# stattlab/azplugins

Hardware: AMD Instinct MI355X
Metric: particle-steps/sec, PerturbedLennardJones pair force (higher is better)
Workload: dtype f64

## Files before the change

### azplugins_amd/csrc/azp_device.hpp

```cpp
#pragma once

#include <hip/hip_runtime.h>
#include <stdint.h>

#include "../../include/azp.h"

namespace azp
{
constexpr int WAVE = 64;

struct BoxDev
    {
    double Lx, Ly, Lz;
    double Lxinv, Lyinv, Lzinv;
    double xy, xz, yz;
    int px, py, pz;
    int triclinic;
    };

inline BoxDev make_box_dev(const azp_box& b)
    {
    BoxDev d;
    d.Lx = b.L[0]; d.Ly = b.L[1]; d.Lz = b.L[2];
    d.Lxinv = 1.0 / b.L[0]; d.Lyinv = 1.0 / b.L[1]; d.Lzinv = 1.0 / b.L[2];
// ... 116 lines not shown
    {
    if (TPP >= 2) v += dpp_move<0xB1>(v);
    if (TPP >= 4) v += dpp_move<0x4E>(v);
    if (TPP >= 8) v += dpp_move<0x141>(v);
    if (TPP >= 16) v += dpp_move<0x140>(v);
    if (TPP >= 32) v += __shfl_xor(v, 16, WAVE);
    if (TPP >= 64) v += __shfl_xor(v, 32, WAVE);
    return v;
    }

__device__ __forceinline__ uint32_t wave_inclusive_scan(uint32_t v)
    {
    const uint32_t lane = threadIdx.x & (WAVE - 1);
#pragma unroll
    for (uint32_t d = 1; d < WAVE; d <<= 1)
        {
        const uint32_t up = (uint32_t)__shfl_up((int)v, d, WAVE);
        if (lane >= d)
            v += up;
        }
    return v;
    }

template<uint32_t NW> __device__ __forceinline__ uint32_t block_exclusive_scan(uint32_t mine, uint32_t* s_wave, uint32_t& total)
    {
    const uint32_t lane = threadIdx.x & (WAVE - 1), wave = threadIdx.x / WAVE;
    const uint32_t incl = wave_inclusive_scan(mine);
    if (lane == WAVE - 1)
        s_wave[wave] = incl;
    __syncthreads();
    uint32_t before = 0;
    total = 0;
#pragma unroll
    for (uint32_t w = 0; w < NW; ++w)
        {
        const uint32_t x = s_wave[w];
        before += (w < wave) ? x : 0u;
        total += x;
        }
    return before + (incl - mine);
    }

__device__ __forceinline__ double fast_rcp(double a)
    {
    const double x = __builtin_amdgcn_rcp(a);
    const double e = __builtin_fma(-a, x, 1.0);
    const double t = __builtin_fma(e, e, e);
    return __builtin_fma(x, t, x);
    }

__device__ __forceinline__ double fast_rcp1(double a)
    {
    const double x = __builtin_amdgcn_rcp(a);
    const double e = __builtin_fma(-a, x, 1.0);
    return __builtin_fma(x, e, x);
    }

__device__ __forceinline__ double fast_rsqrt(double a)
    {
    const double y = __builtin_amdgcn_rsq(a);
    const double h = __builtin_fma(-a * y, y, 1.0);
    return __builtin_fma(y * h, __builtin_fma(0.375, h, 0.5), y);
    }
__device__ __forceinline__ double fast_sqrt(double a)
    {
    const double s = a * fast_rsqrt(a);
    return (a > 0.0) ? s : 0.0;
    }

template<class T> __device__ __forceinline__ T to_uniform(const T& v)
    {
    static_assert(sizeof(T) % 4 == 0, "to_uniform needs whole dwords");
    constexpr int W = sizeof(T) / 4;
    uint32_t w[W];
    __builtin_memcpy(w, &v, sizeof(T));
#pragma unroll
    for (int i = 0; i < W; ++i)
        w[i] = (uint32_t)__builtin_amdgcn_readfirstlane((int)w[i]);
    T r;
    __builtin_memcpy(&r, w, sizeof(T));
    return r;
    }

__device__ __forceinline__ uint32_t xcd_remap(uint32_t b, uint32_t nblocks_padded8)
    {
    const uint32_t per_xcd = nblocks_padded8 >> 3;
    return (b & 7u) * per_xcd + (b >> 3);
    }

}
```

### azplugins_amd/csrc/pair_kernel.hpp

```cpp
#pragma once

#include <type_traits>

#include "evaluators.hpp"
#include "pair_kernel_host.hpp"

namespace azp
{
struct PairKArgs
    {
    double* force;
    double* virial;
    uint64_t virial_pitch;
    const double* pos;
    const uint32_t* n_neigh;
    const uint32_t* nlist;
    const uint64_t* head_list;
    const double* rcutsq;
    const double* ronsq;
    BoxDev box;
    double r_list_max;
    uint32_t N;
    uint32_t ntypes;
    uint32_t shift_mode;
    uint32_t nblocks_padded;
    uint32_t first;
    uint32_t end;
    };

template<class E> __device__ __forceinline__ typename E::Coeff
prepare_coeff(const PairKArgs& a, const typename E::Params* params, uint32_t tp)
    {
    const double rcutsq = a.rcutsq[tp];
    bool energy_shift = (a.shift_mode == AZP_SHIFT_SHIFT);
    if (a.shift_mode == AZP_SHIFT_XPLOR && a.ronsq[tp] > rcutsq)
        energy_shift = true;
    return E::prepare(params[tp], rcutsq, energy_shift);
    }

inline int validate_pair_args(const azp_pair_args* args, const void* d_params)
    {
    if (!args || !d_params) return AZP_ERROR_INVALID_ARGUMENT;
    if (args->N == 0) return 1;
    if (!args->d_force || !args->d_pos || !args->d_n_neigh || !args->d_nlist || !args->d_head_list || !args->d_rcutsq)
        return AZP_ERROR_INVALID_ARGUMENT;
    if (args->ntypes == 0 || args->shift_mode > AZP_SHIFT_XPLOR) return AZP_ERROR_INVALID_ARGUMENT;
    if (args->shift_mode == AZP_SHIFT_XPLOR && !args->d_ronsq) return AZP_ERROR_INVALID_ARGUMENT;
    if (args->compute_virial && (!args->d_virial || args->virial_pitch < args->N)) return AZP_ERROR_INVALID_ARGUMENT;
    if (args->n_max < args->N) return AZP_ERROR_INVALID_ARGUMENT;
    if (args->block_size && (args->block_size % 64 || args->block_size > 256)) return AZP_ERROR_INVALID_ARGUMENT;
    if (args->range_count && (uint64_t)args->range_first + args->range_count > args->N) return AZP_ERROR_INVALID_ARGUMENT;
    return 0;
    }

struct ForceEnergy
    {
    struct Acc
        {
        double fx, fy, fz, pe;
        };
    static __device__ __forceinline__ void zero(Acc& a) { a.fx = a.fy = a.fz = a.pe = 0.0; }
    template<int TPP> static __device__ __forceinline__ void reduce(Acc& a)
        {
        a.fx = group_sum<TPP>(a.fx);
        a.fy = group_sum<TPP>(a.fy);
        a.fz = group_sum<TPP>(a.fz);
        a.pe = group_sum<TPP>(a.pe);
        }
    template<class KExtra> static __device__ __forceinline__ void store(const Acc& a, const PairKArgs& p, const KExtra&, uint32_t idx)
        {
        store_scalar4(p.force, idx, a.fx, a.fy, a.fz, 0.5 * a.pe);
        }
    };

template<class E, bool XPLOR = false> struct XIso : ForceEnergy
    {
    typedef typename E::Params Params;
    struct Coeff
        {
        typename E::Coeff c;
        double ronsq;
        };
    struct KExtra {};
    struct Own {};
    static constexpr int kExtra = 0;
    static constexpr bool kTag = false;
    static __device__ __forceinline__ Coeff prepare(const Params* params, const PairKArgs& a, uint32_t t, const KExtra&)
        {
        Coeff c;
        c.c = prepare_coeff<E>(a, params, t);
        c.ronsq = XPLOR ? a.ronsq[t] : 0.0;
        return c;
        }
    static __device__ __forceinline__ void load_own(const KExtra&, uint32_t, Own&) {}
    static __device__ __forceinline__ void load_extra(const KExtra&, uint32_t, const double*, uint32_t&) {}
    static __device__ __forceinline__ bool in_range(const Coeff&, double) { return true; }
    template<bool VIRIAL>
    static __device__ __forceinline__ void pair(const Coeff& c, const KExtra&, const Own&, double dx, double dy, double dz, double rsq,
                                                const double*, uint32_t, Acc& a, double (&v)[6])
        {
        double force_divr, pair_eng;
        const bool evaluated = E::eval(c.c, rsq, force_divr, pair_eng);
        if (XPLOR && evaluated)
            apply_xplor(rsq, c.ronsq, c.c.rcutsq, force_divr, pair_eng);
        a.fx = __builtin_fma(dx, force_divr, a.fx);
        a.fy = __builtin_fma(dy, force_divr, a.fy);
        a.fz = __builtin_fma(dz, force_divr, a.fz);
        a.pe += pair_eng;
        if (VIRIAL)
            {
            const double fxx = force_divr * dx, fyy = force_divr * dy;
            v[0] = __builtin_fma(fxx, dx, v[0]);
            v[1] = __builtin_fma(fxx, dy, v[1]);
            v[2] = __builtin_fma(fxx, dz, v[2]);
            v[3] = __builtin_fma(fyy, dy, v[3]);
            v[4] = __builtin_fma(fyy, dz, v[4]);
            v[5] = __builtin_fma(force_divr * dz, dz, v[5]);
            }
// ... 219 lines not shown
```

### azplugins_amd/csrc/pair_plj.hip

```cpp
#include "pair_auto.hpp"

extern "C" int azp_pair_forces_perturbed_lennard_jones(const azp_pair_args* args, const azp_plj_params* d_params, void* stream)
    {
    return azp::launch_policy_entry<azp::XIso<azp::EvalPLJ>>(args, d_params, stream);
    }

extern "C" int azp_pair_forces_planned_perturbed_lennard_jones(azp_pair_plan* plan, const azp_pair_args* args,
                                                const azp_plj_params* d_params, void* stream)
    {
    return azp::launch_policy_planned<azp::XIso<azp::EvalPLJ>>(plan, args, d_params, stream);
    }

#ifdef AZP_TIMELINE
namespace azp { __device__ unsigned long long g_timeline[8 * 4 * 16384]; }
extern "C" int azp_debug_timeline(unsigned long long* out, size_t n_words)
    {
    return (int)hipMemcpyFromSymbol(out, HIP_SYMBOL(azp::g_timeline), n_words * sizeof(unsigned long long));
    }
#endif
```

### azplugins_amd/csrc/pair_tiled.hpp

```cpp
#pragma once

#include <type_traits>

#include "pair_kernel.hpp"
#include "pair_plan.hpp"

#ifndef AZP_TILED_WAVES_PER_SIMD
#define AZP_TILED_WAVES_PER_SIMD 4
#endif

namespace azp
{
#ifdef AZP_TIMELINE
extern __device__ unsigned long long g_timeline[8 * 4 * 16384];
#endif

struct TileDyn
    {
    uint32_t n_shells;
    uint32_t stale;
    };

struct TiledKArgs
    {
    PairKArgs p;
    const uint32_t* tile_nstage;
    const uint64_t* tile_head;
    const uint32_t* stage_idx;
    const uint32_t* slice_Kend;
    uint32_t n_shells;
    const uint64_t* slice_head;
    const uint4* cnl;
    const uint8_t* perm;
    const TileDyn* dyn;
    const uint32_t* dflag;
    const unsigned long long* dbits;
    const float* disp;
    double shell_w;
    double shell_winv;
    double bound_extra;
    };

__device__ __forceinline__ float wave_max_nonneg(float v)
    {
#pragma unroll
    for (int off = 32; off > 0; off >>= 1)
        v = fmaxf(v, __shfl_xor(v, off, 64));
    return v;
    }

__device__ __forceinline__ uint32_t tile_shells_for(double b, double shell_winv)
    {
    if (!(b >= 0.0))
        return PLAN_SHELLS;
    if (b == 0.0)
        return 0u;
    if (!(shell_winv > 0.0))
        return PLAN_SHELLS;
    const double n = ceil(2.0 * b * (1.0 + 1e-9) * shell_winv);
    return n >= (double)PLAN_SHELLS ? PLAN_SHELLS : (uint32_t)n;
    }

#define AZP_TILE_STRIDE(CAP) ((CAP) + 1)

constexpr int TILE_BATCH = 4;

struct TileBatch
    {
    double x[TILE_BATCH], y[TILE_BATCH], z[TILE_BATCH];
    uint32_t off[TILE_BATCH];
    };

inline void fill_local_bound(TiledKArgs& k, const PairPlan& plan, const azp_pair_args& args)
    {
    const bool local = args.d_displacement && args.has_displacement_bound && args.displacement_bound >= 0.0;
    k.disp = local ? args.d_displacement : nullptr;
    k.dflag = (args.d_stale_flag && args.d_displacement_sq_bits) ? args.d_stale_flag : nullptr;
    k.dbits = k.dflag ? args.d_displacement_sq_bits : nullptr;
    if (k.dflag)
        k.disp = nullptr;
    k.shell_w = plan.shell_width;
    k.shell_winv = plan.shell_width > 0.0 ? 1.0 / plan.shell_width : 0.0;
    k.bound_extra = args.displacement_bound_extra > 0.0 ? args.displacement_bound_extra : 0.0;
    }

template<int CAP, int H> __device__ __forceinline__ void tile_gather(TileBatch& b, const uint4& u, const char* bx)
    {
    constexpr int NB = TILE_BATCH;
    const uint32_t w0 = H ? u.z : u.x, w1 = H ? u.w : u.y;
    b.off[0] = w0 & 0xffffu;
    b.off[1] = w0 >> 16;
    b.off[2] = w1 & 0xffffu;
    b.off[3] = w1 >> 16;
#pragma unroll
    for (int e = 0; e < NB; ++e)
        {
        b.x[e] = *reinterpret_cast<const double*>(bx + b.off[e]);
// ... 10 lines not shown
                                             double& fz, double& pe, double (&v)[6], uint32_t& n_core, uint32_t& n_in, double (&es)[2])
    {
    typedef typename E::Coeff Coeff;
    constexpr int NB = TILE_BATCH;
    constexpr bool SPLIT = SINGLE && !XPLOR && E::kSplitEnergy;
    double dx[NB], dy[NB], dz[NB], rsq[NB];
    bool any_in = false;
#pragma unroll
    for (int e = 0; e < NB; ++e)
        {
        dx[e] = pi.x - b.x[e]; dy[e] = pi.y - b.y[e]; dz[e] = pi.z - b.z[e];
        if (WRAP)
            min_image(a.p.box, dx[e], dy[e], dz[e]);
        rsq[e] = __builtin_fma(dz[e], dz[e], __builtin_fma(dy[e], dy[e], dx[e] * dx[e]));
        if (WRAP)
            rsq[e] = (b.off[e] == 0) ? 1.0e60 : rsq[e];
        any_in = any_in || (rsq[e] < rcutsq_max);
        }
    const bool none_in = !__any(any_in);
    if (SPLIT ? __builtin_expect(none_in, 0) : none_in)
        return;
    double fd[NB];
    if constexpr (SPLIT)
        {
        double x[NB];
        E::rcp4(rsq, x);
        bool any_core = false;
#pragma unroll
        for (int e = 0; e < NB; ++e)
            any_core = any_core || E::in_core(c0, rsq[e]);
        if (!__any(any_core))
            {
            const bool count_in = c0.tail_add != 0.0;
#pragma unroll
            for (int e = 0; e < NB; ++e)
                E::eval_split_tail(c0, rsq[e], x[e], fd[e], es[0], es[1], n_in, count_in);
            }
        else
            {
#pragma unroll
            for (int e = 0; e < NB; ++e)
                E::eval_split(c0, rsq[e], x[e], fd[e], pe, n_core, n_in);
            }
        }
#pragma unroll
    for (int e = 0; e < NB; ++e)
        {
        double force_divr, pair_eng = 0.0;
        if constexpr (SPLIT)
            force_divr = fd[e];
        else if (SINGLE)
            {
            const bool evaluated = E::eval(c0, rsq[e], force_divr, pair_eng);
            if (XPLOR && evaluated)
                apply_xplor(rsq[e], ronsq0, c0.rcutsq, force_divr, pair_eng);
            }
        else
            {
            const int typej = *reinterpret_cast<const int*>(bt + (b.off[e] >> 1));
            const uint32_t tp = (uint32_t)typei * a.p.ntypes + (uint32_t)typej;
            const Coeff cc = s_coeff[tp];
            const bool evaluated = E::eval(cc, rsq[e], force_divr, pair_eng);
            if (XPLOR && evaluated)
                apply_xplor(rsq[e], s_ronsq[tp], cc.rcutsq, force_divr, pair_eng);
            }
        fx = __builtin_fma(dx[e], force_divr, fx);
        fy = __builtin_fma(dy[e], force_divr, fy);
        fz = __builtin_fma(dz[e], force_divr, fz);
        if constexpr (!SPLIT)
            pe += pair_eng;
        if (VIRIAL)
            {
            const double fxx = force_divr * dx[e], fyy = force_divr * dy[e];
            v[0] = __builtin_fma(fxx, dx[e], v[0]);
            v[1] = __builtin_fma(fxx, dy[e], v[1]);
            v[2] = __builtin_fma(fxx, dz[e], v[2]);
            v[3] = __builtin_fma(fyy, dy[e], v[3]);
            v[4] = __builtin_fma(fyy, dz[e], v[4]);
            v[5] = __builtin_fma(force_divr * dz[e], dz[e], v[5]);
            }
        }
    }

template<class E, int TPP, int CAP, bool VIRIAL, bool SINGLE, bool XPLOR, bool WRAP>
__device__ __forceinline__ void tiled_loop(const TiledKArgs& a, const char* bx, const char* bt,
                                           const typename E::Coeff* __restrict__ s_coeff,
                                           const double* __restrict__ s_ronsq, const typename E::Coeff& c0, double ronsq0,
                                           double rcutsq_max, const char* __restrict__ slice_base, uint32_t lane_off, uint32_t Kb,
                                           double3 pi, int typei, double& fx, double& fy, double& fz, double& pe, double (&v)[6], uint32_t& n_core,
                                           uint32_t& n_in, double (&es)[2])
    {
    const uint4 zero4 = make_uint4(0, 0, 0, 0);
    auto chunk_at = [&](uint32_t kk) -> uint4
        { return *reinterpret_cast<const uint4*>(slice_base + (uint64_t)kk * 1024u + lane_off); };
    const uint32_t K = Kb >> 1;
    const uint32_t Kc = (Kb + 1u) >> 1;
    uint4 u = (Kc > 0) ? chunk_at(0) : zero4;
    uint4 un = (Kc > 1) ? chunk_at(1) : u;
    TileBatch A, B;
    tile_gather<CAP, 0>(A, u, bx);
    for (uint32_t kk = 0; kk < K; ++kk)
        {
        const uint4 un2 = chunk_at((kk + 2 < Kc) ? kk + 2 : Kc - 1);
        tile_gather<CAP, 1>(B, u, bx);
        __builtin_amdgcn_sched_barrier(0);
        tile_compute<E, CAP, VIRIAL, SINGLE, XPLOR, WRAP>(A, a, bt, s_coeff, s_ronsq, c0, ronsq0, rcutsq_max, pi, typei, fx, fy, fz, pe, v, n_core, n_in, es);
        __builtin_amdgcn_sched_barrier(0);
        tile_gather<CAP, 0>(A, un, bx);
        __builtin_amdgcn_sched_barrier(0);
        tile_compute<E, CAP, VIRIAL, SINGLE, XPLOR, WRAP>(B, a, bt, s_coeff, s_ronsq, c0, ronsq0, rcutsq_max, pi, typei, fx, fy, fz, pe, v, n_core, n_in, es);
        __builtin_amdgcn_sched_barrier(0);
        u = un;
        un = un2;
        }
    if (Kb & 1u)
        tile_compute<E, CAP, VIRIAL, SINGLE, XPLOR, WRAP>(A, a, bt, s_coeff, s_ronsq, c0, ronsq0, rcutsq_max, pi, typei, fx, fy, fz, pe, v, n_core, n_in, es);
    }

template<class E, int TPP, int CAP, bool VIRIAL, bool SINGLE, bool XPLOR>
__global__ void __launch_bounds__(256, E::kTileWaves) pair_forces_tiled_kernel(const TiledKArgs a, const typename E::Params* __restrict__ params)
    {
    typedef typename E::Coeff Coeff;
    constexpr int TB = 256 / TPP;
    constexpr int PW = 64 / TPP;
    extern __shared__ __attribute__((aligned(16))) unsigned char s_raw[];
    double* s_x = reinterpret_cast<double*>(s_raw);
    double* s_y = s_x + AZP_TILE_STRIDE(CAP);
    double* s_z = s_y + AZP_TILE_STRIDE(CAP);
    int* s_t = reinterpret_cast<int*>(s_z + AZP_TILE_STRIDE(CAP));
    Coeff* s_coeff = reinterpret_cast<Coeff*>(s_raw + (size_t)AZP_TILE_STRIDE(CAP) * 24 + (SINGLE ? 0 : (size_t)CAP * 4 + 8));
    double* s_ronsq = reinterpret_cast<double*>(s_coeff + (SINGLE ? 0 : a.p.ntypes * a.p.ntypes));

    const uint32_t tid = threadIdx.x;
    __builtin_amdgcn_s_setprio(3);
#ifdef AZP_TIMELINE
    const unsigned long long tl_t0 = __builtin_amdgcn_s_memrealtime();
    const unsigned long long tl_c0 = __builtin_amdgcn_s_memtime();
    unsigned long long tl_tb = 0, tl_tc = 0, tl_td = 0, tl_ta = 0;
#endif
    const uint32_t tile = a.p.first / TB + xcd_remap(blockIdx.x, a.p.nblocks_padded);
    const uint32_t first = tile * TB;
    if (first >= a.p.end)
        return;
    if (a.dyn && a.dyn->stale)
        return;
    if (a.dflag && *a.dflag)
        return;

    Coeff c0;
    double ronsq0 = 0.0;
    double rcutsq_max = 0.0;
    if (SINGLE)
        {
        c0 = to_uniform(prepare_coeff<E>(a.p, params, 0));
        if (XPLOR)
            ronsq0 = a.p.ronsq[0];
        rcutsq_max = c0.rcutsq;
        }
    else
        {
        const uint32_t ntp = a.p.ntypes * a.p.ntypes;
        for (uint32_t t = tid; t < ntp; t += 256)
            {
            s_coeff[t] = prepare_coeff<E>(a.p, params, t);
            s_ronsq[t] = XPLOR ? a.p.ronsq[t] : 0.0;
            }
        for (uint32_t t = 0; t < ntp; ++t)
            rcutsq_max = fmax(rcutsq_max, a.p.rcutsq[t]);
        }

#ifdef AZP_TIMELINE
    tl_ta = __builtin_amdgcn_s_memrealtime();
#endif
    const uint32_t n_stage = a.tile_nstage[tile];
    const uint32_t* __restrict__ stage = a.stage_idx + a.tile_head[tile];
    const double3 c = load_scalar3_of4(a.p.pos, first);
    if (tid == 0)
        {
        s_x[0] = PLAN_FAR; s_y[0] = PLAN_FAR; s_z[0] = PLAN_FAR;
        if (!SINGLE) s_t[0] = 0;
        }
    const uint32_t wave = (uint32_t)__builtin_amdgcn_readfirstlane((int)(tid >> 6)), lane = tid & 63;
    const uint32_t pl = lane / TPP;
    const uint32_t idx = first + ((TPP == 1 && a.perm) ? (uint32_t)a.perm[(uint64_t)tile * 256u + tid] : wave * PW + pl);
    const bool active = idx < a.p.end;
    const double4 own = load_scalar4(a.p.pos, active ? idx : first);
    const bool no_hint = !(a.p.r_list_max > 0.0);
    bool far_from_c = false;
    float dmax = a.disp ? a.disp[active ? idx : first] : 0.f;
    {
    constexpr int ROUNDS = (CAP + 255) / 256;
    uint32_t sj[ROUNDS];
#pragma unroll
    for (int r = 0; r < ROUNDS; ++r)
        {
        const uint32_t sidx = (uint32_t)r * 256u + tid;
        sj[r] = (sidx < n_stage) ? stage[sidx] : first;
        }
#ifdef AZP_TIMELINE
    __builtin_amdgcn_s_waitcnt(0);
    tl_tb = __builtin_amdgcn_s_memrealtime();
#endif
    double sxv[ROUNDS], syv[ROUNDS], szv[ROUNDS];
    int stv[ROUNDS];
    if (a.disp)
        {
#pragma unroll
        for (int r = 0; r < ROUNDS; ++r)
            dmax = fmaxf(dmax, a.disp[sj[r]]);
        }
#pragma unroll
    for (int r = 0; r < ROUNDS; ++r)
        {
        if (SINGLE)
            {
            const double3 pj = load_scalar3_of4(a.p.pos, sj[r]);
            sxv[r] = pj.x; syv[r] = pj.y; szv[r] = pj.z;
            }
        else
            {
            const double4 pj = load_scalar4(a.p.pos, sj[r]);
            sxv[r] = pj.x; syv[r] = pj.y; szv[r] = pj.z;
            stv[r] = type_from_w(pj.w);
            }
        }
#ifdef AZP_TIMELINE
    __builtin_amdgcn_s_waitcnt(0);
    tl_tc = __builtin_amdgcn_s_memrealtime();
#endif
#pragma unroll
    for (int r = 0; r < ROUNDS; ++r)
        {
        const uint32_t sidx = (uint32_t)r * 256u + tid;
        if (sidx < n_stage)
            {
            double x = sxv[r], y = syv[r], z = szv[r];
            if (!a.p.box.triclinic)
                {
                if (a.p.box.px) x = __builtin_fma(-a.p.box.Lx, rint((x - c.x) * a.p.box.Lxinv), x);
                if (a.p.box.py) y = __builtin_fma(-a.p.box.Ly, rint((y - c.y) * a.p.box.Lyinv), y);
                if (a.p.box.pz) z = __builtin_fma(-a.p.box.Lz, rint((z - c.z) * a.p.box.Lzinv), z);
                if (no_hint)
                    far_from_c = far_from_c || (a.p.box.px && fabs(x - c.x) >= 0.25 * a.p.box.Lx)
                                 || (a.p.box.py && fabs(y - c.y) >= 0.25 * a.p.box.Ly)
                                 || (a.p.box.pz && fabs(z - c.z) >= 0.25 * a.p.box.Lz);
                }
            s_x[sidx + 1] = x; s_y[sidx + 1] = y; s_z[sidx + 1] = z;
            if (!SINGLE)
                s_t[sidx + 1] = stv[r];
            }
        }
    }

    double3 pi = make_double3(0.0, 0.0, 0.0);
    int typei = 0;
    bool lane_wide = far_from_c || a.p.box.triclinic;
    if (active)
        {
        const double4 p = own;
        double x = p.x, y = p.y, z = p.z;
        if (!a.p.box.triclinic)
            {
            if (a.p.box.px) x = __builtin_fma(-a.p.box.Lx, rint((x - c.x) * a.p.box.Lxinv), x);
            if (a.p.box.py) y = __builtin_fma(-a.p.box.Ly, rint((y - c.y) * a.p.box.Lyinv), y);
            if (a.p.box.pz) z = __builtin_fma(-a.p.box.Lz, rint((z - c.z) * a.p.box.Lzinv), z);
            const double rx = no_hint ? 0.25 * a.p.box.Lx : a.p.r_list_max, ry = no_hint ? 0.25 * a.p.box.Ly : a.p.r_list_max,
                         rz = no_hint ? 0.25 * a.p.box.Lz : a.p.r_list_max;
            lane_wide = lane_wide || (a.p.box.px && fabs(x - c.x) + rx >= 0.5 * a.p.box.Lx)
                        || (a.p.box.py && fabs(y - c.y) + ry >= 0.5 * a.p.box.Ly)
                        || (a.p.box.pz && fabs(z - c.z) + rz >= 0.5 * a.p.box.Lz);
            }
        pi = make_double3(x, y, z);
        typei = type_from_w(p.w);
        }
#ifdef AZP_TIMELINE
    __builtin_amdgcn_s_waitcnt(0);
    tl_td = __builtin_amdgcn_s_memrealtime();
#endif
    __shared__ float s_dmax[4];
    if (a.disp)
        {
        dmax = wave_max_nonneg(dmax);
        if (lane == 0)
            s_dmax[wave] = dmax;
        }
    const bool wide = __syncthreads_or(lane_wide);
    __builtin_amdgcn_s_setprio(0);
#ifdef AZP_TIMELINE
    const unsigned long long tl_t1 = __builtin_amdgcn_s_memrealtime();
#endif
    uint32_t n_shells = a.dyn ? min(a.dyn->n_shells, PLAN_SHELLS) : a.n_shells;
    if (a.dbits)
        n_shells = tile_shells_for(to_uniform(sqrt(__longlong_as_double((long long)*a.dbits)) + a.bound_extra), a.shell_winv);
    if (a.disp)
        {
        const float d4 = fmaxf(fmaxf(s_dmax[0], s_dmax[1]), fmaxf(s_dmax[2], s_dmax[3]));
        n_shells = tile_shells_for(to_uniform((double)d4 + a.bound_extra), a.shell_winv);
        }

    const uint32_t slice = tile * 4 + wave;
    const uint32_t Kb = to_uniform(a.slice_Kend[(PLAN_SHELLS + 1) * slice + min(n_shells, PLAN_SHELLS)]);
    const uint64_t slice_head = to_uniform(a.slice_head[slice]);
    const char* __restrict__ slice_base = reinterpret_cast<const char*>(a.cnl + slice_head * 64ull);
    const uint32_t lane_off = lane * 16u;

    double fx = 0.0, fy = 0.0, fz = 0.0, pe = 0.0;
    double v[6] = {0.0, 0.0, 0.0, 0.0, 0.0, 0.0};
    uint32_t n_core = 0, n_in = 0;
    double es[2] = {0.0, 0.0};
    const char* bx = reinterpret_cast<const char*>(s_x);
    const char* bt = reinterpret_cast<const char*>(s_t);
    if (wide)
        tiled_loop<E, TPP, CAP, VIRIAL, SINGLE, XPLOR, true>(a, bx, bt, s_coeff, s_ronsq, c0, ronsq0, rcutsq_max, slice_base, lane_off, Kb, pi,
                                                            typei, fx, fy, fz, pe, v, n_core, n_in, es);
    else
        tiled_loop<E, TPP, CAP, VIRIAL, SINGLE, XPLOR, false>(a, bx, bt, s_coeff, s_ronsq, c0, ronsq0, rcutsq_max, slice_base, lane_off, Kb, pi,
                                                             typei, fx, fy, fz, pe, v, n_core, n_in, es);
    if constexpr (SINGLE && !XPLOR && E::kSplitEnergy)
        pe = E::finish_split(c0, pe, es[0], es[1], n_core, n_in);

#ifdef AZP_TIMELINE
    if (lane == 0 && tile < 16384)
        {
        unsigned long long* t = g_timeline + (tile * 4 + wave) * 8;
        t[4] = tl_ta; t[5] = tl_tb; t[6] = tl_tc; t[7] = tl_td;
        if (wave == 3)
            t[4] = __builtin_amdgcn_s_memtime() - tl_c0;
        t[0] = tl_t0; t[1] = tl_t1; t[2] = __builtin_amdgcn_s_memrealtime();
        t[3] = ((unsigned long long)__builtin_amdgcn_s_getreg((20 ) | (0 << 6) | (31 << 11)) << 32)
               | (unsigned)__builtin_amdgcn_s_getreg((4 ) | (0 << 6) | (31 << 11));
        }
#endif
    fx = group_sum<TPP>(fx);
    fy = group_sum<TPP>(fy);
    fz = group_sum<TPP>(fz);
    pe = group_sum<TPP>(pe);
    if (VIRIAL)
        {
#pragma unroll
        for (int cidx = 0; cidx < 6; ++cidx)
            v[cidx] = group_sum<TPP>(v[cidx]);
        }
    if (active && (lane % TPP) == 0)
        {
        store_scalar4(a.p.force, idx, fx, fy, fz, 0.5 * pe);
        if (VIRIAL)
            {
#pragma unroll
            for (int cidx = 0; cidx < 6; ++cidx)
                a.p.virial[(uint64_t)cidx * a.p.virial_pitch + idx] = 0.5 * v[cidx];
            }
        }
    }

inline TiledKArgs make_tiled_kargs(const PairPlan& plan, const azp_pair_args& args, const TileDyn* dyn, uint32_t tb)
    {
    TiledKArgs k = {};
    k.p = make_pair_kargs(args);
    k.tile_nstage = plan.d_tile_nstage;
    k.tile_head = plan.d_tile_head;
    k.stage_idx = plan.d_stage_idx;
    k.perm = plan.balanced ? plan.d_perm : nullptr;
    k.slice_Kend = plan.d_slice_Kend;
    k.n_shells = plan_shells_for(plan, args);
    fill_local_bound(k, plan, args);
    k.dyn = dyn;
    k.slice_head = plan.d_slice_head;
    k.cnl = plan.d_cnl;
    const uint32_t t0 = k.p.first / tb, t1 = (k.p.end + tb - 1) / tb;
    k.p.first = t0 * tb;
    k.p.end = (t1 * tb < args.N) ? t1 * tb : args.N;
    k.p.nblocks_padded = (t1 - t0 + 7u) & ~7u;
    return k;
    }

inline uint32_t plan_launch_cap(const PairPlan& plan, const azp_pair_args& args, uint32_t tb)
    {
    if (args.range_count == 0 || plan.h_tile_nstage.empty())
        return plan.cap;
    const uint32_t end = (args.range_first + args.range_count < args.N) ? args.range_first + args.range_count : args.N;
    const uint32_t t0 = args.range_first / tb, t1 = (end + tb - 1) / tb;
    uint32_t most = 0;
    for (uint32_t t = t0; t < t1 && t < plan.n_tiles; ++t)
        most = plan.h_tile_nstage[t] > most ? plan.h_tile_nstage[t] : most;
    return plan_cap_for(most);
    }

template<class E, int TPP, int CAP, bool VIRIAL, bool SINGLE>
int launch_tiled_instance(const PairPlan& plan, const azp_pair_args& args, const typename E::Params* d_params,
                          hipStream_t stream, const TileDyn* dyn)
    {
    const TiledKArgs k = make_tiled_kargs(plan, args, dyn, plan.tile);
    size_t lds = (size_t)AZP_TILE_STRIDE(CAP) * 24 + (SINGLE ? 0 : (size_t)CAP * 4 + 8);
    if (!SINGLE)
        lds += (sizeof(typename E::Coeff) + sizeof(double)) * (size_t)args.ntypes * args.ntypes;
    if (args.shift_mode == AZP_SHIFT_XPLOR)
        return launch_dyn_lds(pair_forces_tiled_kernel<E, TPP, CAP, VIRIAL, SINGLE, true>, k.p.nblocks_padded, 256, TPP, lds, stream, k, d_params);
    return launch_dyn_lds(pair_forces_tiled_kernel<E, TPP, CAP, VIRIAL, SINGLE, false>, k.p.nblocks_padded, 256, TPP, lds, stream, k, d_params);
    }

template<class E, int TPP, bool VIRIAL, bool SINGLE>
int launch_tiled_cap(const PairPlan& plan, const azp_pair_args& args, const typename E::Params* d_params, hipStream_t s, const TileDyn* dyn)
    {
    const uint32_t cap = plan_launch_cap(plan, args, plan.tile);
    switch (cap)
        {
    case 1024: return launch_tiled_instance<E, TPP, 1024, VIRIAL, SINGLE>(plan, args, d_params, s, dyn);
    case 1536: return launch_tiled_instance<E, TPP, 1536, VIRIAL, SINGLE>(plan, args, d_params, s, dyn);
// ... 31 lines not shown
```

### azplugins_amd/csrc/xtiled.hpp

```cpp
#pragma once

#include <type_traits>

#include "pair_tiled.hpp"

namespace azp
{
template<class X, bool SINGLE> __host__ __device__ constexpr size_t xtiled_lds_slots(size_t cap)
    {
    return cap * (24 + 8 * (size_t)X::kExtra + (X::kTag ? 4 : 0) + (SINGLE ? 0 : 4));
    }

template<class X, int CAP, bool VIRIAL, bool SINGLE>
__global__ void __launch_bounds__(256, X::kMinWaves) xtiled_kernel(const TiledKArgs a, const typename X::KExtra x, const typename X::Params* __restrict__ params)
    {
    typedef typename X::Coeff Coeff;
    constexpr int NE = X::kExtra;
    extern __shared__ __attribute__((aligned(16))) unsigned char s_raw[];
    double* s_pos = reinterpret_cast<double*>(s_raw);
    double* s_ext = s_pos + 3 * CAP;
    uint32_t* s_tag = reinterpret_cast<uint32_t*>(s_ext + NE * CAP);
    int* s_type = reinterpret_cast<int*>(s_tag + (X::kTag ? CAP : 0));
    Coeff* s_coeff = reinterpret_cast<Coeff*>(s_raw + xtiled_lds_slots<X, SINGLE>(CAP));

    const uint32_t tid = threadIdx.x;
    const uint32_t tile = a.p.first / 256u + xcd_remap(blockIdx.x, a.p.nblocks_padded);
    const uint32_t first = tile * 256u;
    if (first >= a.p.end)
        return;
    if (a.dyn && a.dyn->stale)
        return;
    if (a.dflag && *a.dflag)
        return;

    Coeff c0;
    if (SINGLE)
        c0 = to_uniform(X::prepare(params, a.p, 0, x));
    else
        {
        const uint32_t ntp = a.p.ntypes * a.p.ntypes;
        for (uint32_t t = tid; t < ntp; t += 256)
            s_coeff[t] = X::prepare(params, a.p, t, x);
        }

    const uint32_t n_stage = a.tile_nstage[tile];
    const uint32_t* __restrict__ stage = a.stage_idx + a.tile_head[tile];
    const double3 c = load_scalar3_of4(a.p.pos, first);
    if (tid == 0)
        {
        s_pos[0] = PLAN_FAR; s_pos[CAP] = PLAN_FAR; s_pos[2 * CAP] = PLAN_FAR;
#pragma unroll
        for (int e = 0; e < NE; ++e)
            s_ext[e * CAP] = 0.0;
        if (X::kTag) s_tag[0] = 0;
        if (!SINGLE) s_type[0] = 0;
        }
    const uint32_t wave = (uint32_t)__builtin_amdgcn_readfirstlane((int)(tid >> 6)), lane = tid & 63;
    const uint32_t idx = first + (a.perm ? (uint32_t)a.perm[(uint64_t)tile * 256u + tid] : wave * 64u + lane);
    const bool active = idx < a.p.end;
    const bool no_hint = !(a.p.r_list_max > 0.0);
    bool lane_wide = a.p.box.triclinic;
    float dmax = a.disp ? a.disp[active ? idx : first] : 0.f;
    __builtin_amdgcn_s_setprio(3);
    {
    constexpr int ROUNDS = (CAP + 255) / 256;
    uint32_t sj[ROUNDS];
#pragma unroll
    for (int r = 0; r < ROUNDS; ++r)
        {
        const uint32_t sidx = (uint32_t)r * 256u + tid;
        sj[r] = (sidx < n_stage) ? stage[sidx] : first;
        }
    double4 pj[ROUNDS];
    double ext[ROUNDS][NE];
    uint32_t tagj[ROUNDS];
    if (a.disp)
        {
#pragma unroll
        for (int r = 0; r < ROUNDS; ++r)
            dmax = fmaxf(dmax, a.disp[sj[r]]);
        }
#pragma unroll
    for (int r = 0; r < ROUNDS; ++r)
        {
        pj[r] = load_scalar4(a.p.pos, sj[r]);
        tagj[r] = 0;
        X::load_extra(x, sj[r], ext[r], tagj[r]);
        }
#pragma unroll
    for (int r = 0; r < ROUNDS; ++r)
        {
        const uint32_t sidx = (uint32_t)r * 256u + tid;
        if (sidx < n_stage)
            {
            double px = pj[r].x, py = pj[r].y, pz = pj[r].z;
            if (!a.p.box.triclinic)
                {
                if (a.p.box.px) px = __builtin_fma(-a.p.box.Lx, rint((px - c.x) * a.p.box.Lxinv), px);
                if (a.p.box.py) py = __builtin_fma(-a.p.box.Ly, rint((py - c.y) * a.p.box.Lyinv), py);
                if (a.p.box.pz) pz = __builtin_fma(-a.p.box.Lz, rint((pz - c.z) * a.p.box.Lzinv), pz);
                if (no_hint)
                    lane_wide = lane_wide || (a.p.box.px && fabs(px - c.x) >= 0.25 * a.p.box.Lx)
                                || (a.p.box.py && fabs(py - c.y) >= 0.25 * a.p.box.Ly) || (a.p.box.pz && fabs(pz - c.z) >= 0.25 * a.p.box.Lz);
                }
            s_pos[sidx + 1] = px; s_pos[CAP + sidx + 1] = py; s_pos[2 * CAP + sidx + 1] = pz;
#pragma unroll
            for (int e = 0; e < NE; ++e)
                s_ext[e * CAP + sidx + 1] = ext[r][e];
            if (X::kTag) s_tag[sidx + 1] = tagj[r];
            if (!SINGLE) s_type[sidx + 1] = type_from_w(pj[r].w);
            }
        }
    }

    double3 pi = make_double3(0.0, 0.0, 0.0);
    int typei = 0;
    typename X::Own own;
    X::load_own(x, active ? idx : first, own);
    if (active)
        {
        const double4 p = load_scalar4(a.p.pos, idx);
        double px = p.x, py = p.y, pz = p.z;
        if (!a.p.box.triclinic)
            {
            if (a.p.box.px) px = __builtin_fma(-a.p.box.Lx, rint((px - c.x) * a.p.box.Lxinv), px);
            if (a.p.box.py) py = __builtin_fma(-a.p.box.Ly, rint((py - c.y) * a.p.box.Lyinv), py);
            if (a.p.box.pz) pz = __builtin_fma(-a.p.box.Lz, rint((pz - c.z) * a.p.box.Lzinv), pz);
            const double rx = no_hint ? 0.25 * a.p.box.Lx : a.p.r_list_max, ry = no_hint ? 0.25 * a.p.box.Ly : a.p.r_list_max,
                         rz = no_hint ? 0.25 * a.p.box.Lz : a.p.r_list_max;
            lane_wide = lane_wide || (a.p.box.px && fabs(px - c.x) + rx >= 0.5 * a.p.box.Lx) || (a.p.box.py && fabs(py - c.y) + ry >= 0.5 * a.p.box.Ly)
                        || (a.p.box.pz && fabs(pz - c.z) + rz >= 0.5 * a.p.box.Lz);
            }
        pi = make_double3(px, py, pz);
        typei = type_from_w(p.w);
        }
    __shared__ float s_dmax[4];
    if (a.disp)
        {
        dmax = wave_max_nonneg(dmax);
        if (lane == 0)
            s_dmax[wave] = dmax;
        }
    const bool wide = __syncthreads_or(lane_wide);
    __builtin_amdgcn_s_setprio(0);
    uint32_t n_shells = a.dyn ? min(a.dyn->n_shells, PLAN_SHELLS) : a.n_shells;
    if (a.dbits)
        n_shells = tile_shells_for(to_uniform(sqrt(__longlong_as_double((long long)*a.dbits)) + a.bound_extra), a.shell_winv);
    if (a.disp)
        n_shells = tile_shells_for(to_uniform((double)fmaxf(fmaxf(s_dmax[0], s_dmax[1]), fmaxf(s_dmax[2], s_dmax[3])) + a.bound_extra), a.shell_winv);

    const uint32_t slice = tile * 4 + wave;
    const uint32_t K = (to_uniform(a.slice_Kend[(PLAN_SHELLS + 1) * slice + min(n_shells, PLAN_SHELLS)]) + 1u) >> 1;
    const uint64_t slice_head = to_uniform(a.slice_head[slice]);
    const uint4* __restrict__ rows = a.cnl + slice_head * 64ull + lane;

    typename X::Acc acc;
    X::zero(acc);
    double v[6] = {0.0, 0.0, 0.0, 0.0, 0.0, 0.0};
    double rcutsq_max = 0.0;
    if (SINGLE)
        rcutsq_max = c0.rcutsq;
    else
        for (uint32_t t = 0; t < a.p.ntypes * a.p.ntypes; ++t)
            rcutsq_max = fmax(rcutsq_max, a.p.rcutsq[t]);

    auto walk = [&](auto wide_tag)
        {
        constexpr bool WIDE = decltype(wide_tag)::value;
        uint4 u = (K > 0) ? rows[0] : make_uint4(0, 0, 0, 0);
        for (uint32_t kk = 0; kk < K; ++kk)
            {
            const uint4 un = rows[(uint64_t)((kk + 1 < K) ? kk + 1 : kk) * 64u];
            const uint32_t w[4] = {u.x, u.y, u.z, u.w};
            uint32_t slot[8];
            double dx[8], dy[8], dz[8], rsq[8];
            bool any_in = false;
#pragma unroll
            for (int e = 0; e < 8; ++e)
                {
                slot[e] = ((e & 1) ? (w[e >> 1] >> 16) : (w[e >> 1] & 0xffffu)) >> 3;
                dx[e] = pi.x - s_pos[slot[e]];
                dy[e] = pi.y - s_pos[CAP + slot[e]];
                dz[e] = pi.z - s_pos[2 * CAP + slot[e]];
                if (WIDE)
                    min_image(a.p.box, dx[e], dy[e], dz[e]);
                rsq[e] = __builtin_fma(dz[e], dz[e], __builtin_fma(dy[e], dy[e], dx[e] * dx[e]));
                if (WIDE)
                    rsq[e] = (slot[e] == 0) ? 1.0e60 : rsq[e];
                any_in = any_in || !(rsq[e] > rcutsq_max);
                }
            if (__any(any_in))
                {
#pragma unroll
                for (int e = 0; e < 8; ++e)
                    {
                    Coeff cc;
                    if (SINGLE)
                        cc = c0;
                    else
                        cc = s_coeff[(uint32_t)typei * a.p.ntypes + (uint32_t)s_type[slot[e]]];
                    if (X::in_range(cc, rsq[e]))
                        {
                        double ext[NE];
#pragma unroll
                        for (int q = 0; q < NE; ++q)
                            ext[q] = s_ext[q * CAP + slot[e]];
                        const uint32_t tagj = X::kTag ? s_tag[slot[e]] : 0u;
                        X::template pair<VIRIAL>(cc, x, own, dx[e], dy[e], dz[e], rsq[e], ext, tagj, acc, v);
                        }
                    }
                }
            u = un;
            }
        };
    if (wide)
        walk(std::true_type());
    else
        walk(std::false_type());
    if (active)
        {
        X::store(acc, a.p, x, idx);
        if (VIRIAL)
            {
#pragma unroll
            for (int cidx = 0; cidx < 6; ++cidx)
                a.p.virial[(uint64_t)cidx * a.p.virial_pitch + idx] = 0.5 * v[cidx];
            }
        }
    }

template<class X, int CAP, bool VIRIAL, bool SINGLE>
int launch_xtiled_instance(const PairPlan& plan, const azp_pair_args& args, const typename X::KExtra& x, const typename X::Params* d_params,
                           hipStream_t stream, const TileDyn* dyn)
    {
    const TiledKArgs k = make_tiled_kargs(plan, args, dyn, 256);
    size_t lds = xtiled_lds_slots<X, SINGLE>(CAP);
    if (!SINGLE)
// ... 36 lines not shown
```

Measured before the change: 9.045 billion.

## Hoist tile header loads to scalar path and prefetch first neighbor chunk early

Per-tile headers (stage count, stage head, slice head, batch end) are now read through constant-address-space scalar loads at kernel entry instead of after the staging phase. The first neighbor-list chunk is also prefetched before coefficient preparation, so its latency overlaps with staging. Coefficient loads in the single-type path use scalar loads as well. This moves several dependent global loads off the critical path, at the cost of speculatively loading a chunk that may be replaced when the displacement-based shell count differs.

Result: no change. 9.042 billion, median of 2 (-0.0%).

```diff
diff --git a/azplugins_amd/csrc/azp_device.hpp b/azplugins_amd/csrc/azp_device.hpp
--- a/azplugins_amd/csrc/azp_device.hpp
+++ b/azplugins_amd/csrc/azp_device.hpp
@@ -222,6 +222,20 @@
     return r;
     }
 
+template<class T> __device__ __forceinline__ T load_uniform(const T* p)
+    {
+    static_assert(sizeof(T) % 4 == 0, "load_uniform needs whole dwords");
+    return *(const __attribute__((address_space(4))) T*)p;
+    }
+struct PlainLoad
+    {
+    template<class T> __device__ __forceinline__ T operator()(const T* p) const { return *p; }
+    };
+struct UniformLoad
+    {
+    template<class T> __device__ __forceinline__ T operator()(const T* p) const { return load_uniform(p); }
+    };
+
 __device__ __forceinline__ uint32_t xcd_remap(uint32_t b, uint32_t nblocks_padded8)
     {
     const uint32_t per_xcd = nblocks_padded8 >> 3;
diff --git a/azplugins_amd/csrc/pair_kernel.hpp b/azplugins_amd/csrc/pair_kernel.hpp
--- a/azplugins_amd/csrc/pair_kernel.hpp
+++ b/azplugins_amd/csrc/pair_kernel.hpp
@@ -28,12 +28,12 @@
     uint32_t end;
     };
 
-template<class E> __device__ __forceinline__ typename E::Coeff
-prepare_coeff(const PairKArgs& a, const typename E::Params* params, uint32_t tp)
-    {
-    const double rcutsq = a.rcutsq[tp];
+template<class E, class LD = PlainLoad> __device__ __forceinline__ typename E::Coeff
+prepare_coeff(const PairKArgs& a, const typename E::Params* params, uint32_t tp, LD ld = LD())
+    {
+    const double rcutsq = ld(a.rcutsq + tp);
     bool energy_shift = (a.shift_mode == AZP_SHIFT_SHIFT);
-    if (a.shift_mode == AZP_SHIFT_XPLOR && a.ronsq[tp] > rcutsq)
+    if (a.shift_mode == AZP_SHIFT_XPLOR && ld(a.ronsq + tp) > rcutsq)
         energy_shift = true;
     return E::prepare(params[tp], rcutsq, energy_shift);
     }
diff --git a/azplugins_amd/csrc/pair_plj.hip b/azplugins_amd/csrc/pair_plj.hip
--- a/azplugins_amd/csrc/pair_plj.hip
+++ b/azplugins_amd/csrc/pair_plj.hip
@@ -12,7 +12,7 @@
     }
 
 #ifdef AZP_TIMELINE
-namespace azp { __device__ unsigned long long g_timeline[8 * 4 * 16384]; }
+namespace azp { __device__ unsigned long long g_timeline[TL_WORDS * 4 * 16384]; }
 extern "C" int azp_debug_timeline(unsigned long long* out, size_t n_words)
     {
     return (int)hipMemcpyFromSymbol(out, HIP_SYMBOL(azp::g_timeline), n_words * sizeof(unsigned long long));
diff --git a/azplugins_amd/csrc/pair_tiled.hpp b/azplugins_amd/csrc/pair_tiled.hpp
--- a/azplugins_amd/csrc/pair_tiled.hpp
+++ b/azplugins_amd/csrc/pair_tiled.hpp
@@ -12,7 +12,8 @@
 namespace azp
 {
 #ifdef AZP_TIMELINE
-extern __device__ unsigned long long g_timeline[8 * 4 * 16384];
+constexpr int TL_WORDS = 16;
+extern __device__ unsigned long long g_timeline[TL_WORDS * 4 * 16384];
 #endif
 
 struct TileDyn
@@ -189,21 +190,63 @@
         }
     }
 
+__device__ __forceinline__ uint4 tile_chunk_at(const char* __restrict__ slice_base, uint32_t lane_off, uint32_t kk)
+    {
+    return *reinterpret_cast<const uint4*>(slice_base + (uint64_t)kk * 1024u + lane_off);
+    }
+
+__device__ __forceinline__ uint4 tile_first_chunk(const char* __restrict__ slice_base, uint32_t lane_off, uint32_t Kb, const void* valid)
+    {
+    const char* base = (Kb > 0) ? slice_base : reinterpret_cast<const char*>(valid);
+    return *reinterpret_cast<const uint4*>(base + ((Kb > 0) ? lane_off : 0u));
+    }
+__device__ __forceinline__ void tile_chunks(const char* __restrict__ slice_base, uint32_t lane_off, uint32_t Kb, uint4& u, uint4& un)
+    {
+    u = make_uint4(Kb ? u.x : 0u, Kb ? u.y : 0u, Kb ? u.z : 0u, Kb ? u.w : 0u);
+    un = (Kb > 2) ? tile_chunk_at(slice_base, lane_off, 1) : u;
+    }
+
+__device__ __forceinline__ uint32_t tile_shells_of_launch(const TiledKArgs& a)
+    {
+    uint32_t n_shells = a.dyn ? min(load_uniform(&a.dyn->n_shells), PLAN_SHELLS) : a.n_shells;
+    if (a.dbits)
+        n_shells = tile_shells_for(to_uniform(sqrt(__longlong_as_double((long long)load_uniform(a.dbits))) + a.bound_extra), a.shell_winv);
+    return n_shells;
+    }
+__device__ __forceinline__ uint32_t tile_slice_batches(const TiledKArgs& a, uint32_t slice, uint32_t n_shells)
+    {
+    return load_uniform(a.slice_Kend + (PLAN_SHELLS + 1) * slice + min(n_shells, PLAN_SHELLS));
+    }
+
+struct TileHeaders
+    {
+    uint32_t n_stage;
+    uint64_t stage_head;
+    uint64_t slice_head;
+    uint32_t Kb;
+    };
+__device__ __forceinline__ TileHeaders tile_headers(const TiledKArgs& a, uint32_t tile, uint32_t slice)
+    {
+    TileHeaders h;
+    h.n_stage = load_uniform(a.tile_nstage + tile);
+    h.stage_head = load_uniform(a.tile_head + tile);
+    h.slice_head = load_uniform(a.slice_head + slice);
+    h.Kb = tile_slice_batches(a, slice, a.n_shells);
+    asm volatile("" : "+s"(h.n_stage), "+s"(h.stage_head), "+s"(h.slice_head), "+s"(h.Kb));
+    return h;
+    }
+
 template<class E, int TPP, int CAP, bool VIRIAL, bool SINGLE, bool XPLOR, bool WRAP>
 __device__ __forceinline__ void tiled_loop(const TiledKArgs& a, const char* bx, const char* bt,
                                            const typename E::Coeff* __restrict__ s_coeff,
                                            const double* __restrict__ s_ronsq, const typename E::Coeff& c0, double ronsq0,
                                            double rcutsq_max, const char* __restrict__ slice_base, uint32_t lane_off, uint32_t Kb,
-                                           double3 pi, int typei, double& fx, double& fy, double& fz, double& pe, double (&v)[6], uint32_t& n_core,
+                                           uint4 u, uint4 un, double3 pi, int typei, double& fx, double& fy, double& fz, double& pe, double (&v)[6], uint32_t& n_core,
                                            uint32_t& n_in, double (&es)[2])
     {
-    const uint4 zero4 = make_uint4(0, 0, 0, 0);
-    auto chunk_at = [&](uint32_t kk) -> uint4
-        { return *reinterpret_cast<const uint4*>(slice_base + (uint64_t)kk * 1024u + lane_off); };
+    auto chunk_at = [&](uint32_t kk) -> uint4 { return tile_chunk_at(slice_base, lane_off, kk); };
     const uint32_t K = Kb >> 1;
     const uint32_t Kc = (Kb + 1u) >> 1;
-    uint4 u = (Kc > 0) ? chunk_at(0) : zero4;
-    uint4 un = (Kc > 1) ? chunk_at(1) : u;
     TileBatch A, B;
     tile_gather<CAP, 0>(A, u, bx);
     for (uint32_t kk = 0; kk < K; ++kk)
@@ -243,7 +286,7 @@
 #ifdef AZP_TIMELINE
     const unsigned long long tl_t0 = __builtin_amdgcn_s_memrealtime();
     const unsigned long long tl_c0 = __builtin_amdgcn_s_memtime();
-    unsigned long long tl_tb = 0, tl_tc = 0, tl_td = 0, tl_ta = 0;
+    unsigned long long tl_tb = 0, tl_tc = 0, tl_td = 0, tl_ta = 0, tl_te = 0, tl_tf = 0;
 #endif
     const uint32_t tile = a.p.first / TB + xcd_remap(blockIdx.x, a.p.nblocks_padded);
     const uint32_t first = tile * TB;
@@ -254,47 +297,30 @@
     if (a.dflag && *a.dflag)
         return;
 
-    Coeff c0;
-    double ronsq0 = 0.0;
-    double rcutsq_max = 0.0;
-    if (SINGLE)
-        {
-        c0 = to_uniform(prepare_coeff<E>(a.p, params, 0));
-        if (XPLOR)
-            ronsq0 = a.p.ronsq[0];
-        rcutsq_max = c0.rcutsq;
-        }
-    else
-        {
-        const uint32_t ntp = a.p.ntypes * a.p.ntypes;
-        for (uint32_t t = tid; t < ntp; t += 256)
-            {
-            s_coeff[t] = prepare_coeff<E>(a.p, params, t);
-            s_ronsq[t] = XPLOR ? a.p.ronsq[t] : 0.0;
-            }
-        for (uint32_t t = 0; t < ntp; ++t)
-            rcutsq_max = fmax(rcutsq_max, a.p.rcutsq[t]);
-        }
-
-#ifdef AZP_TIMELINE
-    tl_ta = __builtin_amdgcn_s_memrealtime();
-#endif
-    const uint32_t n_stage = a.tile_nstage[tile];
-    const uint32_t* __restrict__ stage = a.stage_idx + a.tile_head[tile];
-    const double3 c = load_scalar3_of4(a.p.pos, first);
-    if (tid == 0)
-        {
-        s_x[0] = PLAN_FAR; s_y[0] = PLAN_FAR; s_z[0] = PLAN_FAR;
-        if (!SINGLE) s_t[0] = 0;
-        }
     const uint32_t wave = (uint32_t)__builtin_amdgcn_readfirstlane((int)(tid >> 6)), lane = tid & 63;
     const uint32_t pl = lane / TPP;
     const uint32_t idx = first + ((TPP == 1 && a.perm) ? (uint32_t)a.perm[(uint64_t)tile * 256u + tid] : wave * PW + pl);
     const bool active = idx < a.p.end;
     const double4 own = load_scalar4(a.p.pos, active ? idx : first);
+    const double3 c = load_scalar3_of4(a.p.pos, first);
+    float dmax = a.disp ? a.disp[active ? idx : first] : 0.f;
+    const uint32_t slice = tile * 4 + wave;
+    const TileHeaders hd = tile_headers(a, tile, slice);
+    const uint32_t n_stage = hd.n_stage;
+    uint32_t Kb = hd.Kb;
+    const uint32_t* __restrict__ stage = a.stage_idx + hd.stage_head;
+    const char* __restrict__ slice_base = reinterpret_cast<const char*>(a.cnl + hd.slice_head * 64ull);
+    const uint32_t lane_off = lane * 16u;
+#ifdef AZP_TIMELINE
+    __builtin_amdgcn_s_waitcnt(0xc07f);
+    tl_ta = __builtin_amdgcn_s_memrealtime();
+#endif
     const bool no_hint = !(a.p.r_list_max > 0.0);
     bool far_from_c = false;
-    float dmax = a.disp ? a.disp[active ? idx : first] : 0.f;
+    uint4 u = make_uint4(0, 0, 0, 0), un;
+    Coeff c0;
+    double ronsq0 = 0.0;
+    double rcutsq_max = 0.0;
     {
     constexpr int ROUNDS = (CAP + 255) / 256;
     uint32_t sj[ROUNDS];
@@ -330,6 +356,35 @@
             sxv[r] = pj.x; syv[r] = pj.y; szv[r] = pj.z;
             stv[r] = type_from_w(pj.w);
             }
+        }
+    if (!a.disp)
+        {
+        if (a.dyn || a.dbits)
+            Kb = tile_slice_batches(a, slice, tile_shells_of_launch(a));
+        u = tile_first_chunk(slice_base, lane_off, Kb, a.p.pos + 4ull * first);
+        }
+    if (SINGLE)
+        {
+        c0 = to_uniform(prepare_coeff<E>(a.p, params, 0, UniformLoad()));
+        if (XPLOR)
+            ronsq0 = load_uniform(a.p.ronsq);
+        rcutsq_max = c0.rcutsq;
+        }
+    else
+        {
+        const uint32_t ntp = a.p.ntypes * a.p.ntypes;
+        for (uint32_t t = tid; t < ntp; t += 256)
+            {
+            s_coeff[t] = prepare_coeff<E>(a.p, params, t);
+            s_ronsq[t] = XPLOR ? a.p.ronsq[t] : 0.0;
+            }
+        for (uint32_t t = 0; t < ntp; ++t)
+            rcutsq_max = fmax(rcutsq_max, load_uniform(a.p.rcutsq + t));
+        }
+    if (tid == 0)
+        {
+        s_x[0] = PLAN_FAR; s_y[0] = PLAN_FAR; s_z[0] = PLAN_FAR;
+        if (!SINGLE) s_t[0] = 0;
         }
 #ifdef AZP_TIMELINE
     __builtin_amdgcn_s_waitcnt(0);
@@ -396,20 +451,19 @@
 #ifdef AZP_TIMELINE
     const unsigned long long tl_t1 = __builtin_amdgcn_s_memrealtime();
 #endif
-    uint32_t n_shells = a.dyn ? min(a.dyn->n_shells, PLAN_SHELLS) : a.n_shells;
-    if (a.dbits)
-        n_shells = tile_shells_for(to_uniform(sqrt(__longlong_as_double((long long)*a.dbits)) + a.bound_extra), a.shell_winv);
     if (a.disp)
         {
         const float d4 = fmaxf(fmaxf(s_dmax[0], s_dmax[1]), fmaxf(s_dmax[2], s_dmax[3]));
-        n_shells = tile_shells_for(to_uniform((double)d4 + a.bound_extra), a.shell_winv);
-        }
-
-    const uint32_t slice = tile * 4 + wave;
-    const uint32_t Kb = to_uniform(a.slice_Kend[(PLAN_SHELLS + 1) * slice + min(n_shells, PLAN_SHELLS)]);
-    const uint64_t slice_head = to_uniform(a.slice_head[slice]);
-    const char* __restrict__ slice_base = reinterpret_cast<const char*>(a.cnl + slice_head * 64ull);
-    const uint32_t lane_off = lane * 16u;
+        const uint32_t n_shells = tile_shells_for(to_uniform((double)d4 + a.bound_extra), a.shell_winv);
+        Kb = tile_slice_batches(a, slice, n_shells);
+        u = tile_first_chunk(slice_base, lane_off, Kb, a.p.pos + 4ull * first);
+        }
+#ifdef AZP_TIMELINE
+    __builtin_amdgcn_s_waitcnt(0xc07f);
+    tl_te = __builtin_amdgcn_s_memrealtime();
+    __builtin_amdgcn_s_waitcnt(0);
+    tl_tf = __builtin_amdgcn_s_memrealtime();
+#endif
 
     double fx = 0.0, fy = 0.0, fz = 0.0, pe = 0.0;
     double v[6] = {0.0, 0.0, 0.0, 0.0, 0.0, 0.0};
@@ -418,19 +472,26 @@
     const char* bx = reinterpret_cast<const char*>(s_x);
     const char* bt = reinterpret_cast<const char*>(s_t);
     if (wide)
-        tiled_loop<E, TPP, CAP, VIRIAL, SINGLE, XPLOR, true>(a, bx, bt, s_coeff, s_ronsq, c0, ronsq0, rcutsq_max, slice_base, lane_off, Kb, pi,
+        {
+        uint4 uw = tile_first_chunk(slice_base, lane_off, Kb, a.p.pos + 4ull * first), uwn;
+        tile_chunks(slice_base, lane_off, Kb, uw, uwn);
+        tiled_loop<E, TPP, CAP, VIRIAL, SINGLE, XPLOR, true>(a, bx, bt, s_coeff, s_ronsq, c0, ronsq0, rcutsq_max, slice_base, lane_off, Kb, uw, uwn, pi,
                                                             typei, fx, fy, fz, pe, v, n_core, n_in, es);
+        }
     else
-        tiled_loop<E, TPP, CAP, VIRIAL, SINGLE, XPLOR, false>(a, bx, bt, s_coeff, s_ronsq, c0, ronsq0, rcutsq_max, slice_base, lane_off, Kb, pi,
+        {
+        tile_chunks(slice_base, lane_off, Kb, u, un);
+        tiled_loop<E, TPP, CAP, VIRIAL, SINGLE, XPLOR, false>(a, bx, bt, s_coeff, s_ronsq, c0, ronsq0, rcutsq_max, slice_base, lane_off, Kb, u, un, pi,
                                                              typei, fx, fy, fz, pe, v, n_core, n_in, es);
+        }
     if constexpr (SINGLE && !XPLOR && E::kSplitEnergy)
         pe = E::finish_split(c0, pe, es[0], es[1], n_core, n_in);
 
 #ifdef AZP_TIMELINE
     if (lane == 0 && tile < 16384)
         {
-        unsigned long long* t = g_timeline + (tile * 4 + wave) * 8;
-        t[4] = tl_ta; t[5] = tl_tb; t[6] = tl_tc; t[7] = tl_td;
+        unsigned long long* t = g_timeline + (tile * 4 + wave) * TL_WORDS;
+        t[4] = tl_ta; t[5] = tl_tb; t[6] = tl_tc; t[7] = tl_td; t[8] = tl_te; t[9] = tl_tf;
         if (wave == 3)
             t[4] = __builtin_amdgcn_s_memtime() - tl_c0;
         t[0] = tl_t0; t[1] = tl_t1; t[2] = __builtin_amdgcn_s_memrealtime();
diff --git a/azplugins_amd/csrc/xtiled.hpp b/azplugins_amd/csrc/xtiled.hpp
--- a/azplugins_amd/csrc/xtiled.hpp
+++ b/azplugins_amd/csrc/xtiled.hpp
@@ -43,8 +43,11 @@
             s_coeff[t] = X::prepare(params, a.p, t, x);
         }
 
-    const uint32_t n_stage = a.tile_nstage[tile];
-    const uint32_t* __restrict__ stage = a.stage_idx + a.tile_head[tile];
+    const uint32_t wave = (uint32_t)__builtin_amdgcn_readfirstlane((int)(tid >> 6)), lane = tid & 63;
+    const uint32_t slice = tile * 4 + wave;
+    const TileHeaders hd = tile_headers(a, tile, slice);
+    const uint32_t n_stage = hd.n_stage;
+    const uint32_t* __restrict__ stage = a.stage_idx + hd.stage_head;
     const double3 c = load_scalar3_of4(a.p.pos, first);
     if (tid == 0)
         {
@@ -55,7 +58,6 @@
         if (X::kTag) s_tag[0] = 0;
         if (!SINGLE) s_type[0] = 0;
         }
-    const uint32_t wave = (uint32_t)__builtin_amdgcn_readfirstlane((int)(tid >> 6)), lane = tid & 63;
     const uint32_t idx = first + (a.perm ? (uint32_t)a.perm[(uint64_t)tile * 256u + tid] : wave * 64u + lane);
     const bool active = idx < a.p.end;
     const bool no_hint = !(a.p.r_list_max > 0.0);
@@ -143,16 +145,13 @@
         }
     const bool wide = __syncthreads_or(lane_wide);
     __builtin_amdgcn_s_setprio(0);
-    uint32_t n_shells = a.dyn ? min(a.dyn->n_shells, PLAN_SHELLS) : a.n_shells;
-    if (a.dbits)
-        n_shells = tile_shells_for(to_uniform(sqrt(__longlong_as_double((long long)*a.dbits)) + a.bound_extra), a.shell_winv);
+    uint32_t Kb = hd.Kb;
     if (a.disp)
-        n_shells = tile_shells_for(to_uniform((double)fmaxf(fmaxf(s_dmax[0], s_dmax[1]), fmaxf(s_dmax[2], s_dmax[3])) + a.bound_extra), a.shell_winv);
-
-    const uint32_t slice = tile * 4 + wave;
-    const uint32_t K = (to_uniform(a.slice_Kend[(PLAN_SHELLS + 1) * slice + min(n_shells, PLAN_SHELLS)]) + 1u) >> 1;
-    const uint64_t slice_head = to_uniform(a.slice_head[slice]);
-    const uint4* __restrict__ rows = a.cnl + slice_head * 64ull + lane;
+        Kb = tile_slice_batches(a, slice, tile_shells_for(to_uniform((double)fmaxf(fmaxf(s_dmax[0], s_dmax[1]), fmaxf(s_dmax[2], s_dmax[3])) + a.bound_extra), a.shell_winv));
+    else if (a.dyn || a.dbits)
+        Kb = tile_slice_batches(a, slice, tile_shells_of_launch(a));
+    const uint32_t K = (Kb + 1u) >> 1;
+    const uint4* __restrict__ rows = a.cnl + hd.slice_head * 64ull + lane;
 
     typename X::Acc acc;
     X::zero(acc);
```
